# Ighina/MultimodalTopicSegmentation

Hardware: NVIDIA B200
Metric: segmented sentences/sec (higher is better)
Workload: dtype f32

## Files before the change

### include/mts_b200.h

```cpp
#ifndef MTS_B200_H_
#define MTS_B200_H_

#include <stdint.h>

#ifdef __cplusplus
extern "C" {
#endif

#define MTS_E_BADARG (-1)
#define MTS_E_UNSUPPORTED (-2)
#define MTS_E_NODEVICE (-3)

int mts_version(void);
const char *mts_last_error(void);
int mts_device_ok(void);


int mts_pack_rows_split(const float *src1, int64_t bstride1, int D1, const float *src2, int64_t bstride2, int D2,
                        int B, int T, int Kp, float *hi, float *lo, void *stream);

int mts_split_tf32(const float *src, int64_t ld, int rows, int cols, int Kp, int side, float *hi, float *lo,
                   void *stream);

int mts_transpose_split(const float *src, int64_t bstride, int64_t ld, int rows, int cols, int T, int shift,
                        const int32_t *lengths, int Kp, int side, float *hi, float *lo, void *stream);

int mts_gather_pad(const float *src, const int64_t *offsets, const int32_t *lengths, const int32_t *ids, int B, int T,
                   int D, float pad, float *out, void *stream);

int mts_ragged_copy(const float *src, float *dst, const int32_t *lengths, const int32_t *offsets, int B, int S, int d,
                    int to_padded, float pad, void *stream);

int mts_gemm_tf32x3(const float *A_hi, const float *A_lo, const float *B_hi, const float *B_lo, const float *bias,
                    float *C, int M, int N, int Kp, int64_t ldc, int epilogue, int accumulate, void *stream);
int mts_gemm_f32(const float *A, int64_t lda, const float *B, int64_t ldb, const float *bias, float *C, int64_t ldc,
                 int M, int N, int K, int layout, int epilogue, int accumulate, int splits, int shift, int T,
                 const int32_t *lengths, void *stream);
int64_t mts_colsum_ws_bytes(int M, int N);
int mts_colsum(const float *X, int64_t ld, int M, int N, float *out, int accumulate, void *ws, void *stream);

int mts_lstm_rec_fwd(const float *gx, const float *w_hh, const int32_t *lengths, const int32_t *order, int n_enc,
                     int B, int T, int H, float *y, float *gates, void *stream);

int mts_lstm_rec_fwd_tc(const float *gx, const float *w_hh, const int32_t *lengths, const int32_t *order, int n_enc,
                        int B, int T, int H, float *y, float *gates, float *y_corr, void *stream);
int mts_lstm_rec_fwd_tf32(const float *gx, const float *w_hh, const int32_t *lengths, const int32_t *order, int n_enc,
                          int B, int T, int H, float *y, float *gates, float *y_corr, void *stream);

int mts_gemm_tf32x3_srcs(const float *A1, int D1, int64_t ld1, const float *A2, int D2, int64_t ld2, const float *A_lo,
                         const float *B_hi, const float *B_lo, const float *bias, float *C, int M, int N, int Kp, int64_t ldc,
                         int epilogue, int accumulate, void *stream);

int mts_pack_rows_f16(const float *src1, int64_t bstride1, int D1, const float *src2, int64_t bstride2, int D2, int B, int T,
                      int K64, void *pieces, float *row_scale, void *stream);
int mts_gemm_f16x3(const void *A_pieces, const void *B_pieces, const float *row_scale, const float *col_scale, const float *bias,
                   float *C, float *C_lo, int M, int N, int K, int64_t ldc, int epilogue, void *stream);

int mts_gemm_tf32x3_gelu_pair(const float *A_hi, const float *A_lo, const float *B_hi, const float *B_lo, const float *bias,
                              float *C, float *C_lo, int M, int N, int Kp, void *stream);

int mts_lstm_rec_fwd_tc_bf16(const float *gx, const float *w_hh, const int32_t *lengths, const int32_t *order, int n_enc,
                             int B, int T, int H, float *y, float *gates, float *y_corr, void *stream);
int mts_gemm_bf16p(const float *A_lo, const float *B_lo, const float *bias, float *C, int M, int N, int Kp, int64_t ldc,
                   int epilogue, int accumulate, void *stream);
int mts_pack_rows_bf16in(const void *src1, int64_t bstride1, int D1, const void *src2, int64_t bstride2, int D2, int B, int T,
                         int Kp, float *lo, void *stream);

int mts_debug_rec_profile(long long *buf);

int mts_lstm_rec_fwd_h3(const float *gx, const float *w_hh, const int32_t *lengths, const int32_t *order, int n_enc,
                        int B, int T, int H, float *y, float *gates, float *y_corr, int precision, void *stream);
int mts_debug_rec_profile_h3(long long *buf);

int mts_lstm_rec_fwd_h3p(const float *gx, const float *w_hh, const int32_t *lengths, const int32_t *order, int n_enc,
                         int B, int T, int H, float *y, float *gates, float *y_corr, int precision, void *stream);
int mts_debug_rec_profile_h3p(long long *buf);

int mts_lstm_rec_bwd(const float *dy, const float *gates, const float *w_hh, const float *w_hh_t,
                     const int32_t *lengths, const int32_t *order, int n_enc, int B, int T, int H, float *dgx,
                     void *stream);

int mts_lstm_rec_bwd_tc(const float *dy, const float *gates, const float *w_hh, const int32_t *lengths,
                        const int32_t *order, int n_enc, int B, int T, int H, float *dgx, void *stream);
int mts_lstm_rec_bwd_h3(const float *dy, const float *gates, const float *w_hh, const int32_t *lengths,
                        const int32_t *order, int n_enc, int B, int T, int H, float *dgx, void *stream);
int mts_lstm_rec_bwd_tf32(const float *dy, const float *gates, const float *w_hh, const int32_t *lengths,
                          const int32_t *order, int n_enc, int B, int T, int H, float *dgx, void *stream);

int mts_head_fwd(const float *feats, const float *w, const float *bias, const int32_t *lengths, int B, int T, int F,
                 int n_out, float th, float *scores, uint8_t *tags, void *stream);
int64_t mts_head_bwd_ws_bytes(int B, int T, int F, int n_out);
int mts_head_bwd(const float *d_scores, const float *feats, const float *w, int B, int T, int F, int n_out,
                 float *d_feats, float *d_w, float *d_bias, void *ws, void *stream);

int mts_seg_loss_fwd(const float *scores, const float *target, int64_t ldt, const int32_t *lengths, int B, int T,
                     int kind, float alpha, float gamma, float inv_count, float *loss_out, float *partial,
                     void *stream);
int mts_seg_loss_bwd(const float *scores, const float *target, int64_t ldt, const int32_t *lengths, int B, int T,
                     int kind, float alpha, float gamma, float inv_count, const float *count_dev,
                     const float *grad_out, float *d_scores, void *stream);

int mts_seg_metrics(const uint8_t *tags, int64_t ld_tags, const float *target, int64_t ldt, const int32_t *lengths,
                    int B, int T, int zero_last, int32_t *out, void *stream);

int mts_crf_viterbi(const float *emis, const int32_t *lengths, const float *trans, int B, int L, int C,
                    float *best_score, int32_t *paths, uint32_t *bp_ws, void *stream);
int mts_crf_nll_fwd(const float *emis, const float *tags, int64_t ldt, const int32_t *lengths, const float *trans,
                    int B, int L, int C, float *log_z, float *gold, float *alphas, void *stream);
int mts_crf_nll_bwd(const float *emis, const float *tags, int64_t ldt, const int32_t *lengths, const float *trans,
                    const float *alphas, int B, int L, int C, const float *scale_dev, float *d_emis,
                    float *d_trans, void *stream);

int mts_embed_ln_fwd(const float *x, int64_t x_bstride, const float *pos, const float *typ, const float *gamma,
                     const float *beta, int B, int S, int d, float eps, float *y, float *y_hi, float *y_lo, int Kp,
                     float *sum_out, float *stats, const int32_t *lengths, const int32_t *offsets, void *stream);
int mts_add_ln_fwd(const float *a, const float *res, const float *gamma, const float *beta, int M, int d, float eps,
                   float *y, float *y_hi, float *y_lo, int Kp, float *sum_out, float *stats, void *stream);
int mts_embed_ln_fwd_f16(const float *x, int64_t x_bstride, const float *pos, const float *typ, const float *gamma,
                         const float *beta, int B, int S, int d, float eps, float *y, void *pieces, int K64, float *row_scale,
                         const int32_t *lengths, const int32_t *offsets, void *stream);
int mts_add_ln_fwd_f16(const float *a, const float *res, const float *gamma, const float *beta, int M, int d, float eps, float *y,
                       void *pieces, int K64, float *row_scale, void *stream);
int mts_gelu_split(const float *src, int64_t ld, int rows, int cols, int Kp, float *act, float *hi, float *lo,
                   void *stream);
// ... 37 lines not shown
```

### multimodaltopicsegmentation_b200/_lib.py

```python
from __future__ import annotations

import ctypes
import os
from ctypes import c_float, c_int, c_int64, c_uint64, c_void_p

_HERE = os.path.dirname(os.path.abspath(__file__))
LIB_PATH = os.path.join(_HERE, "libmts_b200.so")
CSRC = os.path.join(_HERE, "csrc")

_P = c_void_p

SIGNATURES = {
    "mts_version": (c_int, []),
    "mts_last_error": (ctypes.c_char_p, []),
    "mts_device_ok": (c_int, []),
    "mts_pack_rows_split": (c_int, [_P, c_int64, c_int, _P, c_int64, c_int, c_int, c_int, c_int, _P, _P, _P]),
    "mts_split_tf32": (c_int, [_P, c_int64, c_int, c_int, c_int, c_int, _P, _P, _P]),
    "mts_transpose_split": (c_int, [_P, c_int64, c_int64, c_int, c_int, c_int, c_int, _P, c_int, c_int, _P, _P, _P]),
    "mts_gather_pad": (c_int, [_P, _P, _P, _P, c_int, c_int, c_int, c_float, _P, _P]),
    "mts_gemm_tf32x3": (c_int, [_P, _P, _P, _P, _P, _P, c_int, c_int, c_int, c_int64, c_int, c_int, _P]),
    "mts_gemm_f32": (c_int, [_P, c_int64, _P, c_int64, _P, _P, c_int64, c_int, c_int, c_int, c_int, c_int, c_int,
                             c_int, c_int, c_int, _P, _P]),
    "mts_colsum_ws_bytes": (c_int64, [c_int, c_int]),
    "mts_colsum": (c_int, [_P, c_int64, c_int, c_int, _P, c_int, _P, _P]),
    "mts_lstm_rec_fwd": (c_int, [_P, _P, _P, _P, c_int, c_int, c_int, c_int, _P, _P, _P]),
    "mts_lstm_rec_fwd_tc": (c_int, [_P, _P, _P, _P, c_int, c_int, c_int, c_int, _P, _P, _P, _P]),
    "mts_lstm_rec_fwd_tc_bf16": (c_int, [_P, _P, _P, _P, c_int, c_int, c_int, c_int, _P, _P, _P, _P]),
    "mts_lstm_rec_fwd_tf32": (c_int, [_P, _P, _P, _P, c_int, c_int, c_int, c_int, _P, _P, _P, _P]),
    "mts_lstm_rec_fwd_h3": (c_int, [_P, _P, _P, _P, c_int, c_int, c_int, c_int, _P, _P, _P, c_int, _P]),
    "mts_gemm_tf32x3_srcs": (c_int, [_P, c_int, c_int64, _P, c_int, c_int64, _P, _P, _P, _P, _P, c_int, c_int, c_int, c_int64, c_int,
                                     c_int, _P]),
    "mts_pack_rows_f16": (c_int, [_P, c_int64, c_int, _P, c_int64, c_int, c_int, c_int, c_int, _P, _P, _P]),
    "mts_gemm_f16x3": (c_int, [_P, _P, _P, _P, _P, _P, _P, c_int, c_int, c_int, c_int64, c_int, _P]),
    "mts_gemm_tf32x3_gelu_pair": (c_int, [_P, _P, _P, _P, _P, _P, _P, c_int, c_int, c_int, _P]),
    "mts_gemm_bf16p": (c_int, [_P, _P, _P, _P, c_int, c_int, c_int, c_int64, c_int, c_int, _P]),
    "mts_pack_rows_bf16in": (c_int, [_P, c_int64, c_int, _P, c_int64, c_int, c_int, c_int, c_int, _P, _P]),
    "mts_debug_rec_profile": (c_int, [_P]),
    "mts_debug_rec_profile_h3": (c_int, [_P]),
    "mts_lstm_rec_fwd_h3p": (c_int, [_P, _P, _P, _P, c_int, c_int, c_int, c_int, _P, _P, _P, c_int, _P]),
    "mts_debug_rec_profile_h3p": (c_int, [_P]),
    "mts_lstm_rec_bwd": (c_int, [_P, _P, _P, _P, _P, _P, c_int, c_int, c_int, c_int, _P, _P]),
    "mts_lstm_rec_bwd_tc": (c_int, [_P, _P, _P, _P, _P, c_int, c_int, c_int, c_int, _P, _P]),
    "mts_lstm_rec_bwd_h3": (c_int, [_P, _P, _P, _P, _P, c_int, c_int, c_int, c_int, _P, _P]),
    "mts_lstm_rec_bwd_tf32": (c_int, [_P, _P, _P, _P, _P, c_int, c_int, c_int, c_int, _P, _P]),
    "mts_head_fwd": (c_int, [_P, _P, _P, _P, c_int, c_int, c_int, c_int, c_float, _P, _P, _P]),
    "mts_head_bwd_ws_bytes": (c_int64, [c_int, c_int, c_int, c_int]),
    "mts_head_bwd": (c_int, [_P, _P, _P, c_int, c_int, c_int, c_int, _P, _P, _P, _P, _P]),
    "mts_seg_loss_fwd": (c_int, [_P, _P, c_int64, _P, c_int, c_int, c_int, c_float, c_float, c_float, _P, _P, _P]),
    "mts_seg_loss_bwd": (c_int, [_P, _P, c_int64, _P, c_int, c_int, c_int, c_float, c_float, c_float, _P, _P, _P, _P]),
    "mts_seg_metrics": (c_int, [_P, c_int64, _P, c_int64, _P, c_int, c_int, c_int, _P, _P]),
    "mts_crf_viterbi": (c_int, [_P, _P, _P, c_int, c_int, c_int, _P, _P, _P, _P]),
    "mts_crf_nll_fwd": (c_int, [_P, _P, c_int64, _P, _P, c_int, c_int, c_int, _P, _P, _P, _P]),
    "mts_crf_nll_bwd": (c_int, [_P, _P, c_int64, _P, _P, _P, c_int, c_int, c_int, _P, _P, _P, _P]),
    "mts_embed_ln_fwd": (c_int, [_P, c_int64, _P, _P, _P, _P, c_int, c_int, c_int, c_float, _P, _P, _P, c_int, _P, _P, _P, _P,
                                 _P]),
    "mts_embed_ln_fwd_f16": (c_int, [_P, c_int64, _P, _P, _P, _P, c_int, c_int, c_int, c_float, _P, _P, c_int, _P, _P, _P, _P]),
    "mts_add_ln_fwd_f16": (c_int, [_P, _P, _P, _P, c_int, c_int, c_float, _P, _P, c_int, _P, _P]),
    "mts_add_ln_fwd": (c_int, [_P, _P, _P, _P, c_int, c_int, c_float, _P, _P, _P, c_int, _P, _P, _P]),
    "mts_gelu_split": (c_int, [_P, c_int64, c_int, c_int, c_int, _P, _P, _P, _P]),
    "mts_band_attn_fwd": (c_int, [_P, c_int64, _P, _P, c_int, c_int, c_int, c_int, c_int, _P, _P, _P, c_int, _P, _P]),
    "mts_band_attn_fwd_mma": (c_int, [_P, c_int64, _P, _P, c_int, c_int, c_int, c_int, c_int, _P, _P, _P, c_int, _P, _P]),
    "mts_band_attn_fwd_simt": (c_int, [_P, c_int64, _P, _P, c_int, c_int, c_int, c_int, c_int, _P, _P, _P, c_int, _P, _P]),
    "mts_band_attn_fwd_tc": (c_int, [_P, c_int64, _P, _P, c_int, c_int, c_int, c_int, c_int, _P, _P, _P, c_int, _P, _P]),
    "mts_band_attn_tc_supported": (c_int, [c_int]),
    "mts_debug_attn_profile": (c_int, [_P]),
    "mts_ln_bwd_ws_bytes": (c_int64, [c_int, c_int]),
    "mts_ln_bwd": (c_int, [_P, _P, _P, _P, c_int, c_int, _P, _P, _P, c_int, _P, _P, _P, _P]),
    "mts_gelu_bwd": (c_int, [_P, _P, c_int, c_int, c_int, _P, _P, _P, _P]),
    "mts_ragged_copy": (c_int, [_P, _P, _P, _P, c_int, c_int, c_int, c_int, c_float, _P]),
    "mts_embed_bwd": (c_int, [_P, c_int, c_int, c_int, _P, _P, _P, _P]),
    "mts_band_attn_bwd": (c_int, [_P, c_int64, _P, _P, _P, _P, _P, c_int, c_int, c_int, c_int, c_int, _P, _P, _P]),
    "mts_band_attn_fwd_dropout": (c_int, [_P, c_int64, _P, _P, c_int, c_int, c_int, c_int, c_int, _P, _P, _P, c_int, _P, c_float,
                                          c_uint64, _P]),
    "mts_band_attn_bwd_dropout": (c_int, [_P, c_int64, _P, _P, _P, _P, _P, c_int, c_int, c_int, c_int, c_int, _P, _P, c_float,
                                          c_uint64, _P]),
}

_lib = None


class MtsError(RuntimeError):
    pass
# ... 33 lines not shown
```

### multimodaltopicsegmentation_b200/csrc/gemm_tc.cu

```cuda
#include <cuda.h>
#include <stdlib.h>

#include "common.cuh"

namespace mts {

constexpr int TC_BM = 128;
constexpr int TC_BK = 32;
constexpr int TC_UMMA_K = 8;
constexpr int TC_THREADS = 192;

template <int BN>
struct TcCfg {
  static constexpr int kStages = (BN == 256) ? 2 : 3;
  static constexpr int kABytes = TC_BM * TC_BK * 4;
  static constexpr int kBBytes = BN * TC_BK * 4;
  static constexpr int kStageBytes = 2 * kABytes + 2 * kBBytes;
  static constexpr int kTmemCols = 2 * BN;
  static constexpr int kAccStride = BN;
  static constexpr int kSmemBytes = kStages * kStageBytes + 1024  + 256  + 4 * 32 * 32 * 4 ;
};

__device__ __forceinline__ uint32_t s_u32(const void *p) { return (uint32_t)__cvta_generic_to_shared(p); }

// ... 648 lines not shown
  static EncodeTiledFn fn = nullptr;
  if (!fn) {
    void *p = nullptr;
    cudaDriverEntryPointQueryResult q;
    if (cudaGetDriverEntryPoint("cuTensorMapEncodeTiled", &p, cudaEnableDefault, &q) == cudaSuccess &&
        q == cudaDriverEntryPointSuccess)
      fn = (EncodeTiledFn)p;
  }
  return fn;
}

static int make_map(CUtensorMap *map, const float *ptr, int rows, int Kp, int box_rows, bool corr = false, int cols = 0,
                    int64_t ld = 0) {
  EncodeTiledFn fn = get_encode_fn();
  if (!fn) { set_error("gemm_tf32x3: cuTensorMapEncodeTiled not available"); return MTS_E_NODEVICE; }
  if (cols == 0) cols = Kp;
  if (ld == 0) ld = Kp;
  cuuint64_t dims[2] = {(cuuint64_t)(corr ? 2 * cols : cols), (cuuint64_t)rows};
  cuuint64_t strides[1] = {(cuuint64_t)ld * sizeof(float)};
  cuuint32_t box[2] = {(cuuint32_t)(corr ? 2 * TC_BK : TC_BK), (cuuint32_t)box_rows};
  cuuint32_t estr[2] = {1, 1};
  CUresult r = fn(map, corr ? CU_TENSOR_MAP_DATA_TYPE_BFLOAT16 : CU_TENSOR_MAP_DATA_TYPE_FLOAT32, 2, (void *)ptr, dims, strides, box, estr,
                  CU_TENSOR_MAP_INTERLEAVE_NONE, CU_TENSOR_MAP_SWIZZLE_128B, CU_TENSOR_MAP_L2_PROMOTION_L2_256B,
                  CU_TENSOR_MAP_FLOAT_OOB_FILL_NONE);
  if (r != CUDA_SUCCESS) { set_error("gemm_tf32x3: cuTensorMapEncodeTiled failed"); return MTS_E_BADARG; }
  return 0;
}

__global__ void __launch_bounds__(256) zero_matrix_kernel(float *__restrict__ C, int M, int N, int64_t ldc) {
  const int64_t total = (int64_t)M * N;
  for (int64_t i = (int64_t)blockIdx.x * blockDim.x + threadIdx.x; i < total; i += (int64_t)gridDim.x * blockDim.x)
    C[(i / N) * ldc + (i % N)] = 0.0f;
}

struct ASources {
  const float *a1; int d1; int64_t ld1;
  const float *a2; int d2; int64_t ld2;
};

template <int BN>
static int launch_tc(const float *A_hi, const float *A_lo, const float *B_hi, const float *B_lo, const float *bias,
                     float *C, int M, int N, int Kp, int64_t ldc, int epilogue, int accumulate, cudaStream_t st,
                     int bf16_only = 0, float *C_lo = nullptr, const ASources *srcs = nullptr, const float *row_scale = nullptr,
                     const float *col_scale = nullptr) {
  using Cfg = TcCfg<BN>;
  const int tiles_m1 = (M + TC_BM - 1) / TC_BM;
  static const char *force = getenv("MTS_GEMM_CLUSTER");
  int CL = tiles_m1 >= 2 ? 2 : 1;
  if (force) {
    const int want = atoi(force);
    if ((want == 1 || want == 2) && tiles_m1 >= want) CL = want;
  }
  static const char *two = getenv("MTS_GEMM_2SM");
  const bool use_2sm = BN == 256 && tiles_m1 >= 2 && !(two && atoi(two) == 0);
  if (use_2sm) CL = 2;
  static const char *bn2_env = getenv("MTS_GEMM_BN2");
  int bn = BN;
  if (use_2sm && !(bn2_env && atoi(bn2_env) == 256) && N % 256 != 0 && (N + 223) / 224 == (N + 255) / 256)
    bn = 224;
  const int tiles_n = (N + bn - 1) / bn;
  CUtensorMap ma_hi, ma_lo, mb_hi, mb_lo;
  int rc;
  CUtensorMap ma_hi2;
  int a_split_kb = 1 << 30;
  if (srcs) {
    if ((rc = make_map(&ma_hi, srcs->a1, M, Kp, TC_BM, false, srcs->d1, srcs->ld1))) return rc;
    ma_hi2 = ma_hi;
    if (srcs->a2) {
      if ((rc = make_map(&ma_hi2, srcs->a2, M, Kp, TC_BM, false, srcs->d2, srcs->ld2))) return rc;
      a_split_kb = srcs->d1 / TC_BK;
    }
  } else {
    if ((rc = make_map(&ma_hi, A_hi, M, Kp, TC_BM, bf16_only == 2, 0, bf16_only == 2 ? 2 * Kp : 0))) return rc;
    ma_hi2 = ma_hi;
  }
  if ((rc = make_map(&ma_lo, A_lo, M, Kp, TC_BM, true, 0, bf16_only == 2 ? 2 * Kp : 0))) return rc;
  if ((rc = make_map(&mb_hi, B_hi, N, Kp, bn / CL, bf16_only == 2, 0, bf16_only == 2 ? 2 * Kp : 0))) return rc;
  if ((rc = make_map(&mb_lo, B_lo, N, Kp, bn / CL, true, 0, bf16_only == 2 ? 2 * Kp : 0))) return rc;
  MTS_PER_DEVICE(bool, attr_set);
  if (!attr_set) {
    MTS_CUDA(cudaFuncSetAttribute(gemm_tf32x3_kernel<BN, 1>, cudaFuncAttributeMaxDynamicSharedMemorySize, Cfg::kSmemBytes));
    MTS_CUDA(cudaFuncSetAttribute(gemm_tf32x3_kernel<BN, 2>, cudaFuncAttributeMaxDynamicSharedMemorySize, Cfg::kSmemBytes));
    MTS_CUDA(cudaFuncSetAttribute(gemm_tf32x3_2sm_kernel<256>, cudaFuncAttributeMaxDynamicSharedMemorySize, Tc2Cfg<256>::kSmemBytes));
    MTS_CUDA(cudaFuncSetAttribute(gemm_tf32x3_2sm_kernel<224>, cudaFuncAttributeMaxDynamicSharedMemorySize, Tc2Cfg<224>::kSmemBytes));
    attr_set = true;
  }
  const int tiles = ((tiles_m1 + CL - 1) / CL) * tiles_n;
  const int slots = kNumSMs / CL;
  int splits = 1;
  const int num_kb = Kp / TC_BK;
  if (epilogue != 2 && !C_lo) {
    if (tiles * 2 <= slots && num_kb >= 32) {
      splits = slots / tiles;
      if (splits > num_kb / 8) splits = num_kb / 8;
    }
    if (num_kb > 96 && splits < (num_kb + 63) / 64) splits = (num_kb + 63) / 64;
    if (splits < 1) splits = 1;
  }
  if (splits > 1 && !accumulate) {
    const int64_t total = (int64_t)M * N;
    const unsigned zg = (unsigned)((total + 255) / 256 < 1184 ? (total + 255) / 256 : 1184);
    zero_matrix_kernel<<<zg, 256, 0, st>>>(C, M, N, ldc);
  }
  const int items = tiles * splits;
  const int grid = (items < slots ? items : slots) * CL;
  cudaLaunchConfig_t cfg = {};
  cfg.gridDim = dim3((unsigned)grid);
// ... 105 lines not shown
```

### multimodaltopicsegmentation_b200/csrc/lstm_rec_h3.cu

```cuda
#include <cooperative_groups.h>
#include <cuda_fp16.h>
#include <stdlib.h>

#include "cluster_utils.cuh"
#include "tcgen05_utils.cuh"

namespace cg = cooperative_groups;

namespace mts {

constexpr int HR_NB = 16;
constexpr int HR_SUB_THREADS = 160;
constexpr int HR_EPI = 128;
constexpr int HR_PIECE_BYTES = 4 * HR_NB * 128;
constexpr int HR_B_BYTES = 2 * HR_PIECE_BYTES;
constexpr int HR_ACT_FLOATS = 4 * HR_NB * 32;
constexpr int HR_TMEM_COLS = 512;
constexpr int HR_W2_COL = 128;
constexpr int HR_ACC_COL = 256;
constexpr int HR_SUB_BYTES = 2 * HR_B_BYTES + HR_ACT_FLOATS * 4 + 1024;
constexpr int HR_HEAD_BYTES = 1024;
static_assert(HR_SUB_BYTES % 1024 == 0, "SWIZZLE_128B operand buffers need 1024-byte alignment");
template <int NT>
constexpr int hr_smem() {
  return (HR_HEAD_BYTES + NT * HR_SUB_BYTES + 1024) > 120 * 1024 ? (HR_HEAD_BYTES + NT * HR_SUB_BYTES + 1024) : 120 * 1024;
}

__host__ __device__ constexpr uint32_t idesc_f16(int M, int N) {
  return (1u << 4) | ((uint32_t)(N >> 3) << 17) | ((uint32_t)(M >> 4) << 24);
}

__device__ __forceinline__ uint32_t h2_bits(float first, float second) {
  const __half2 h = __floats2half2_rn(first, second);
  return *reinterpret_cast<const uint32_t *>(&h);
}
__device__ __forceinline__ float2 h2_floats(uint32_t bits) {
  return __half22float2(*reinterpret_cast<const __half2 *>(&bits));
}
__device__ __forceinline__ void st_async_v4u(uint32_t raddr, uint4 v, uint32_t rbar) {
  asm volatile("st.async.weak.shared::cluster.mbarrier::complete_tx::bytes.v4.b32 [%0], {%1, %2, %3, %4}, [%5];" ::"r"(raddr),
               "r"(v.x), "r"(v.y), "r"(v.z), "r"(v.w), "r"(rbar)
               : "memory");
}
__device__ __forceinline__ void tmem_st16u(uint32_t taddr, const uint32_t (&v)[16]) {
  asm volatile(
      "tcgen05.st.sync.aligned.32x32b.x16.b32 [%0], "
      "{%1, %2, %3, %4, %5, %6, %7, %8, %9, %10, %11, %12, %13, %14, %15, %16};" ::"r"(taddr),
      "r"(v[0]), "r"(v[1]), "r"(v[2]), "r"(v[3]), "r"(v[4]), "r"(v[5]), "r"(v[6]), "r"(v[7]), "r"(v[8]), "r"(v[9]), "r"(v[10]),
      "r"(v[11]), "r"(v[12]), "r"(v[13]), "r"(v[14]), "r"(v[15])
      : "memory");
}

__device__ __forceinline__ void umma_f16_ts_p(uint32_t d_tmem, uint32_t a_tmem, uint32_t b_lo, uint32_t b_hi, uint32_t idesc,
                                              uint32_t acc) {
  asm volatile(
      "{\n\t.reg .pred p;\n\t.reg .b64 bd;\n\t"
      "setp.ne.b32 p, %5, 0;\n\t"
      "mov.b64 bd, {%2, %3};\n\t"
      "tcgen05.mma.cta_group::1.kind::f16 [%0], [%1], bd, %4, p;\n\t}" ::"r"(d_tmem),
      "r"(a_tmem), "r"(b_lo), "r"(b_hi), "r"(idesc), "r"(acc)
      : "memory");
}

constexpr int HR_PROF_STEPS = 4, HR_PROF_SLOTS = 16;
__device__ long long *g_hr_prof = nullptr;
#define HR_STAMP(slot)                                                                     \
  do {                                                                                     \
    if (prof && s >= 8 && s < 8 + HR_PROF_STEPS) prof[(s - 8) * HR_PROF_SLOTS + (slot)] = clock64(); \
  } while (0)

template <bool SAVE, int NT, bool BF16>
__global__ void __cluster_dims__(kCluster, 1, 1) __launch_bounds__(HR_SUB_THREADS * NT, 1)
    lstm_fwd_h3_kernel(const float *__restrict__ gx, const float *__restrict__ w_hh, const int32_t *__restrict__ lengths,
                       const int32_t *__restrict__ order, int B, int T, int n_enc, int n_tiles, int ept,
                       float *__restrict__ y, float *__restrict__ gates, float *__restrict__ y_corr) {
  constexpr bool bf16_mode = BF16;
  extern __shared__ uint8_t smem_raw[];
  uint8_t *smem = reinterpret_cast<uint8_t *>((reinterpret_cast<uintptr_t>(smem_raw) + 1023) & ~(uintptr_t)1023);
  const int tid = threadIdx.x, lane = tid & 31;
  const int warp = __shfl_sync(0xffffffffu, tid >> 5, 0);
  const int sub = (NT == 2 && warp >= 5) ? 1 : 0;
  const int wr = warp - 5 * sub;

  float *rscale_s = reinterpret_cast<float *>(smem);
  uint32_t *tmem_slot = reinterpret_cast<uint32_t *>(smem + 512);
  uint8_t *sub_base = smem + HR_HEAD_BYTES + sub * HR_SUB_BYTES;
  uint8_t *bbuf = sub_base;
  float *act = reinterpret_cast<float *>(bbuf + 2 * HR_B_BYTES);
  uint64_t *bars = reinterpret_cast<uint64_t *>(act + HR_ACT_FLOATS);
  uint64_t *h_full = bars;
  uint64_t *acc_full = bars + 16;
  int *len_s = reinterpret_cast<int *>(bars + 18);
  int *bq_s = len_s + HR_NB;

  cg::cluster_group cluster = cg::this_cluster();
  const uint32_t rank = cluster.block_rank();
  const int n_clusters = gridDim.x / kCluster;
  const int groups = (n_tiles + NT - 1) / NT;
  const int n_items = groups * 2 * n_enc;
  const int ycols = n_enc * 2 * kH;

  if (wr == 0 && lane == 0) {
    for (int i = 0; i < 4; ++i) tc::bar_init(tc::s_u32(&h_full[i]), 1);
    tc::bar_init(tc::s_u32(acc_full), 1);
    asm volatile("fence.mbarrier_init.release.cluster;" ::: "memory");
  }
  if (warp == 0) tc::tmem_alloc<HR_TMEM_COLS>(tc::s_u32(tmem_slot));
  tc::tc_fence_before();
  __syncthreads();
  tc::tc_fence_after();
  const uint32_t tmem_base = *tmem_slot;
  const uint32_t acc_col = HR_ACC_COL + 16 * sub;

  uint32_t ph_h = 0, ph_acc = 0;

  const int et = (wr - 1) * 32 + lane;
  const int q = warp & 3;
  const int cj = et & 7, ce = et >> 3;

  int cur_dir = -1, cur_enc = -1;
  long long *prof = (blockIdx.x == 0 && (tid == 0 || tid == 32)) ? g_hr_prof : nullptr;

  for (int item = blockIdx.x / kCluster; item < n_items; item += n_clusters) {
    const int tile = (item % groups) * NT + sub;
    const int dir = (item / groups) & 1;
    const int enc = item / (2 * groups);
    const float *W = w_hh + ((size_t)enc * 2 + dir) * 4 * kH * kH;

// ... 127 lines not shown
      for (int i = 0; i < kCluster; ++i) {
        const uint32_t r = (rank + i) & 7;
        const uint32_t off = (uint32_t)(piece * HR_PIECE_BYTES + (i >> 1) * (HR_NB * 128) + ce * 128 +
                                        ((((i & 1) * 4 + chunk) ^ (ce & 7)) << 4));
        raddr[i] = mapa(tc::s_u32(bbuf) + off, r);
        rbar[i] = mapa(tc::s_u32(&h_full[i >> 2]), r);
      }
      const bool sender = ce < ept && !(bf16_mode && piece);

      for (int s = 0; s < nsteps; ++s) {
        const int p = s & 1;
        float gxc[HR_NB];
#pragma unroll
        for (int e = 0; e < HR_NB; ++e) {
          gxc[e] = gxn[e];
          const int len = len_s[e];
          if (s + 1 < len) {
            const int tn = dir ? len - 2 - s : s + 1;
            gxn[e] = __ldg(gx + gx_enc + ((size_t)bq_s[e] * T + tn) * 8 * kH + gcol);
          }
        }
        tc::bar_wait_wd(tc::s_u32(acc_full), ph_acc); ph_acc ^= 1;
        HR_STAMP(10);
        tc::tc_fence_after();
        float pre[HR_NB];
        tc::tmem_ld16(tmem_base + ((uint32_t)(q * 32) << 16) + acc_col, pre);
        tc::tc_fence_before();
        HR_STAMP(11);
        const float zs = (q == 2) ? -2.0f * 1.4426950408889634f : -1.4426950408889634f;
        const float oa = (q == 2) ? 2.0f : 1.0f, ob = (q == 2) ? -1.0f : 0.0f;
#define HR_ACT(NCOL)                                                          \
  _Pragma("unroll") for (int e = 0; e < (NCOL); ++e) {                        \
    const float z = fmaf(pre[e], rs, gxc[e]);                                 \
    const float sg = __fdividef(1.0f, 1.0f + exp2f(z * zs));                  \
    act[(q * HR_NB + e) * 32 + lane] = fmaf(sg, oa, ob);                      \
  }
        if (ept > 14) { HR_ACT(16) } else if (ept > 12) { HR_ACT(14) } else if (ept > 10) { HR_ACT(12) } else if (ept > 8) { HR_ACT(10) }
        else if (ept > 6) { HR_ACT(8) } else if (ept > 4) { HR_ACT(6) } else if (ept > 2) { HR_ACT(4) } else { HR_ACT(2) }
#undef HR_ACT
        if (sub == 0) asm volatile("bar.sync 1, 128;" ::: "memory");
        else asm volatile("bar.sync 2, 128;" ::: "memory");
        HR_STAMP(12);
        const float4 ig = *reinterpret_cast<const float4 *>(act + (0 * HR_NB + ce) * 32 + 4 * cj);
        const float4 fg = *reinterpret_cast<const float4 *>(act + (1 * HR_NB + ce) * 32 + 4 * cj);
        const float4 gg = *reinterpret_cast<const float4 *>(act + (2 * HR_NB + ce) * 32 + 4 * cj);
        const float4 og = *reinterpret_cast<const float4 *>(act + (3 * HR_NB + ce) * 32 + 4 * cj);
        float4 hn = make_float4(0.f, 0.f, 0.f, 0.f);
        if (s < my_len) {
          c[0] = fmaf(fg.x, c[0], ig.x * gg.x); c[1] = fmaf(fg.y, c[1], ig.y * gg.y);
          c[2] = fmaf(fg.z, c[2], ig.z * gg.z); c[3] = fmaf(fg.w, c[3], ig.w * gg.w);
          hn = make_float4(og.x * tanh_fast(c[0]), og.y * tanh_fast(c[1]), og.z * tanh_fast(c[2]), og.w * tanh_fast(c[3]));
        }
        HR_STAMP(13);
        if (s + 1 < nsteps) {
          uint32_t p1a, p1b, p2a = 0u, p2b = 0u;
          if (bf16_mode) {
            p1a = bf16x2_bits(hn.x, hn.y);
            p1b = bf16x2_bits(hn.z, hn.w);
          } else {
            p1a = h2_bits(hn.x, hn.y);
            p1b = h2_bits(hn.z, hn.w);
            const float2 f0 = h2_floats(p1a), f1 = h2_floats(p1b);
            p2a = h2_bits(hn.x - f0.x, hn.y - f0.y);
            p2b = h2_bits(hn.z - f1.x, hn.w - f1.y);
          }
          const uint32_t ga = piece ? p1a : p2a, gb = piece ? p1b : p2b;
          const uint32_t ra = __shfl_xor_sync(0xffffffffu, ga, 1), rb = __shfl_xor_sync(0xffffffffu, gb, 1);
          const uint4 gran = piece ? make_uint4(ra, rb, p2a, p2b) : make_uint4(p1a, p1b, ra, rb);
          if (sender) {
            const uint32_t boff = (uint32_t)((p ^ 1) * HR_B_BYTES), moff = (uint32_t)((p ^ 1) * 16);
#pragma unroll
            for (int r = 0; r < kCluster; ++r) st_async_v4u(raddr[r] + boff, gran, rbar[r] + moff);
          }
        }
        HR_STAMP(14);
        if (s < my_len) {
          const int t = dir ? my_len - 1 - s : s;
          *reinterpret_cast<float4 *>(y + ((size_t)my_b * T + t) * ycols + ycol) = hn;
          if (y_corr) corr_store4(y_corr + ((size_t)my_b * T + t) * ycols, (int)ycol, hn, 0);
          if (SAVE) {
            float *gs = gates + ((gate_base + my_b) * T + t) * 5 * kH + rank * kUnits + 4 * cj;
            *reinterpret_cast<float4 *>(gs) = ig;
            *reinterpret_cast<float4 *>(gs + kH) = fg;
            *reinterpret_cast<float4 *>(gs + 2 * kH) = gg;
            *reinterpret_cast<float4 *>(gs + 3 * kH) = og;
            *reinterpret_cast<float4 *>(gs + 4 * kH) = make_float4(c[0], c[1], c[2], c[3]);
          }
        }
      }
      if (my_b >= 0)
        for (int t = my_len; t < T; ++t) {
          const float4 z = make_float4(0.f, 0.f, 0.f, 0.f);
          *reinterpret_cast<float4 *>(y + ((size_t)my_b * T + t) * ycols + ycol) = z;
          if (y_corr) corr_store4(y_corr + ((size_t)my_b * T + t) * ycols, (int)ycol, z, 0);
        }
    }
    tc::tc_fence_before();
    __syncthreads();
    cluster.sync();
  }
  tc::tc_fence_before();
  __syncthreads();
  if (warp == 0) {
    tc::tc_fence_after();
    tc::tmem_dealloc<HR_TMEM_COLS>(tmem_base);
  }
}

template <typename K>
static int h3_max_active_clusters(K kernel, int threads, int smem) {
  cudaLaunchConfig_t cfg = {};
  cfg.gridDim = dim3(kCluster * 64);
  cfg.blockDim = dim3(threads);
  cfg.dynamicSmemBytes = smem;
  cudaLaunchAttribute attr;
  attr.id = cudaLaunchAttributeClusterDimension;
  attr.val.clusterDim.x = kCluster;
  attr.val.clusterDim.y = 1;
  attr.val.clusterDim.z = 1;
  cfg.attrs = &attr;
  cfg.numAttrs = 1;
  int n = 0;
  if (cudaOccupancyMaxActiveClusters(&n, kernel, &cfg) != cudaSuccess || n < 1) {
    cudaGetLastError();
    n = 8;
  }
  return n;
}

}

using namespace mts;

extern "C" int mts_debug_rec_profile_h3(long long *buf) {
  MTS_CUDA(cudaMemcpyToSymbol(g_hr_prof, &buf, sizeof(buf)));
  return 0;
}

template <bool BF16>
static int launch_h3(const float *gx, const float *w_hh, const int32_t *lengths, const int32_t *order, int n_enc, int B, int T,
                     float *y, float *gates, float *y_corr, cudaStream_t st) {
  MTS_PER_DEVICE(int, cap);
  if (!cap) {
    MTS_CUDA(cudaFuncSetAttribute(lstm_fwd_h3_kernel<false, 1, BF16>, cudaFuncAttributeMaxDynamicSharedMemorySize, hr_smem<1>()));
    MTS_CUDA(cudaFuncSetAttribute(lstm_fwd_h3_kernel<true, 1, BF16>, cudaFuncAttributeMaxDynamicSharedMemorySize, hr_smem<1>()));
    MTS_CUDA(cudaFuncSetAttribute(lstm_fwd_h3_kernel<false, 2, BF16>, cudaFuncAttributeMaxDynamicSharedMemorySize, hr_smem<2>()));
    MTS_CUDA(cudaFuncSetAttribute(lstm_fwd_h3_kernel<true, 2, BF16>, cudaFuncAttributeMaxDynamicSharedMemorySize, hr_smem<2>()));
    cap = h3_max_active_clusters(lstm_fwd_h3_kernel<false, 2, BF16>, 2 * HR_SUB_THREADS, hr_smem<2>());
  }
  int ept = HR_NB;
  {
    const int per_dir = cap / (2 * n_enc);
    if (per_dir >= 1 && (B + HR_NB - 1) / HR_NB <= per_dir) {
      const int want = (B + per_dir - 1) / per_dir;
      ept = want < 1 ? 1 : (want > HR_NB ? HR_NB : want);
    }
  }
  static const char *force_ept = getenv("MTS_REC_EPT");
  if (force_ept && atoi(force_ept) >= 1 && atoi(force_ept) <= HR_NB) ept = atoi(force_ept);
  const int n_tiles = (B + ept - 1) / ept;
  const int items1 = n_tiles * 2 * n_enc;
  static const char *force = getenv("MTS_REC_NT");
  const bool two = force ? (force[0] == '2') : (items1 > cap);
  static const char *pair_env = getenv("MTS_REC_PAIR");
  if (pair_env ? (pair_env[0] == '1') : two)
    return mts_lstm_rec_fwd_h3p(gx, w_hh, lengths, order, n_enc, B, T, kH, y, gates, y_corr, BF16 ? 1 : 0, (void *)st);
  if (!two) {
    const unsigned grid = (unsigned)((items1 < cap ? items1 : cap) * kCluster);
    if (gates) lstm_fwd_h3_kernel<true, 1, BF16><<<grid, HR_SUB_THREADS, hr_smem<1>(), st>>>(gx, w_hh, lengths, order, B, T, n_enc, n_tiles, ept, y, gates, y_corr);
    else lstm_fwd_h3_kernel<false, 1, BF16><<<grid, HR_SUB_THREADS, hr_smem<1>(), st>>>(gx, w_hh, lengths, order, B, T, n_enc, n_tiles, ept, y, gates, y_corr);
  } else {
    const int items2 = ((n_tiles + 1) / 2) * 2 * n_enc;
    const unsigned grid = (unsigned)((items2 < cap ? items2 : cap) * kCluster);
    if (gates) lstm_fwd_h3_kernel<true, 2, BF16><<<grid, 2 * HR_SUB_THREADS, hr_smem<2>(), st>>>(gx, w_hh, lengths, order, B, T, n_enc, n_tiles, ept, y, gates, y_corr);
    else lstm_fwd_h3_kernel<false, 2, BF16><<<grid, 2 * HR_SUB_THREADS, hr_smem<2>(), st>>>(gx, w_hh, lengths, order, B, T, n_enc, n_tiles, ept, y, gates, y_corr);
  }
  MTS_LAUNCH_CHECK();
  return 0;
}

extern "C" int mts_lstm_rec_fwd_h3(const float *gx, const float *w_hh, const int32_t *lengths, const int32_t *order, int n_enc,
                                   int B, int T, int H, float *y, float *gates, float *y_corr, int precision, void *stream) {
  MTS_REQUIRE(gx && w_hh && lengths && y, MTS_E_BADARG, "lstm_rec_fwd_h3: null pointer");
  MTS_REQUIRE(n_enc >= 1 && B > 0 && T > 0, MTS_E_BADARG, "lstm_rec_fwd_h3: bad shape");
  MTS_REQUIRE(H == kH, MTS_E_UNSUPPORTED, "lstm_rec_fwd_h3: the tensor-core recurrence serves H == 256");
  MTS_REQUIRE(precision == 0 || precision == 1, MTS_E_BADARG, "lstm_rec_fwd_h3: precision must be 0 (fp16 x3) or 1 (bf16)");
  MTS_REQUIRE(!y_corr || n_enc == 1, MTS_E_UNSUPPORTED, "lstm_rec_fwd_h3: the fused correction operand needs n_enc == 1");
  MTS_REQUIRE((((uintptr_t)y | (uintptr_t)gx | (uintptr_t)w_hh) & 15) == 0, MTS_E_BADARG,
              "lstm_rec_fwd_h3: buffers must be 16-byte aligned");
  cudaStream_t st = (cudaStream_t)stream;
  return precision ? launch_h3<true>(gx, w_hh, lengths, order, n_enc, B, T, y, gates, y_corr, st)
                   : launch_h3<false>(gx, w_hh, lengths, order, n_enc, B, T, y, gates, y_corr, st);
}
```

### multimodaltopicsegmentation_b200/ops.py

```python
from __future__ import annotations

import torch

from . import _lib

_LAUNCHES = 0
_KERNELS_PER_CALL = {
    "mts_seg_loss_fwd": 2, "mts_head_bwd": 3, "mts_colsum": 2, "mts_ln_bwd": 3, "mts_band_attn_bwd": 2,
}


def launch_count():
    return _LAUNCHES


def reset_launch_count():
    global _LAUNCHES
    _LAUNCHES = 0


PROFILE = None
GEMM_IMPL = __import__("os").environ.get("MTS_GEMM_IMPL", "tcgen05")
REC_IMPL = __import__("os").environ.get("MTS_REC_IMPL", "tc")

# ... 311 lines not shown
        cache = ent.setdefault("wih_p", {})
        if e not in cache:
            w_f, _, _, _, w_r = self._params(self.rnns[e], layer)[:5]
            with torch.no_grad():
                cache[e] = f16_pieces_stacked([w_f.detach(), w_r.detach()])
        return cache[e]

    def wih_packed_a(self, layer, e):
        ent = self.get()[layer]
        cache = ent.setdefault("wih_bf", {})
        if e not in cache:
            w_f, _, _, _, w_r = self._params(self.rnns[e], layer)[:5]
            D = w_f.shape[1]
            kp = _pad32(D)
            H4 = w_f.shape[0]
            bf = torch.empty((2, 2 * H4, kp), device=w_f.device, dtype=torch.float32)
            with torch.no_grad():
                for d, w in enumerate((w_f, w_r)):
                    wc = w.detach().contiguous()
                    _call("mts_split_tf32", _ptr(wc), D, H4, D, kp, A_SIDE, _ptr(bf[0, d * H4:]), _ptr(bf[1, d * H4:]), _stream())
            cache[e] = bf[1]
        return cache[e]

    def get(self):
        key = tuple((p.data_ptr(), p._version) for p in self.flat_params())
        if key == self.key:
            return self.layers
        rnn0 = self.rnns[0]
        H, L = rnn0.hidden_size, rnn0.num_layers
        dev = rnn0.weight_hh_l0.device
        layers = []
        with torch.no_grad():
            for layer in range(L):
                wih, bias = [], []
                whh = torch.empty((len(self.rnns), 2, 4 * H, H), device=dev, dtype=torch.float32)
                for e, rnn in enumerate(self.rnns):
                    w_f, h_f, bi_f, bh_f, w_r, h_r, bi_r, bh_r = self._params(rnn, layer)
                    D = w_f.shape[1]
                    kp = _pad32(D)
                    pair = torch.empty((2, 8 * H, kp), device=dev, dtype=torch.float32)
                    for d, w in enumerate((w_f, w_r)):
                        wc = w.detach().contiguous()
                        _call("mts_split_tf32", _ptr(wc), D, 4 * H, D, kp, B_SIDE, _ptr(pair[0, d * 4 * H:]),
                              _ptr(pair[1, d * 4 * H:]), _stream())
                    wih.append((pair[0], pair[1]))
                    bias.append(torch.cat([bi_f.detach() + bh_f.detach(), bi_r.detach() + bh_r.detach()]))
                    whh[e, 0].copy_(h_f.detach())
                    whh[e, 1].copy_(h_r.detach())
                layers.append({"wih": wih, "bias": bias, "whh": whh})
        self.key, self.layers = key, layers
        return layers


def _lstm_stack_forward(x1, x2, xs2, lens, packed, H, L, n_enc, save):
    B, T = lens.B, lens.T
    dev = x1.device
    layers = packed.get()
    saved = []
    y_prev = y_corr = None
    bf16 = PRECISION == "bf16"
    if bf16 and (save or H != 256 or REC_IMPL != "tc" or GEMM_IMPL == "simt"):
        raise NotImplementedError("the bf16 path serves inference with H == 256 on the tensor-core kernels; train in fp32")
    for layer in range(L):
        gx = torch.empty((n_enc, B * T, 8 * H), device=dev, dtype=torch.float32)
        for e in range(n_enc):
            if bf16:
                if layer == 0:
                    a_lo = pack_rows_packed(x1, x2, B, T) if n_enc == 1 else pack_rows_packed(x1 if e == 0 else xs2, None, B, T)
                elif y_corr is not None:
                    a_lo = y_corr
                else:
                    src = y_prev.view(B * T, n_enc * 2 * H)[:, e * 2 * H:(e + 1) * 2 * H]
                    a_lo = split_tf32(src, cols=2 * H, ld=n_enc * 2 * H, rows=B * T)[1]
                _call("mts_gemm_bf16p", _ptr(a_lo), _ptr(packed.wih_packed_a(layer, e)), _ptr(layers[layer]["bias"][e]), _ptr(gx[e]),
                      B * T, 8 * H, a_lo.shape[1], 8 * H, 1, 0, _stream())
                continue
            if layer == 0 and GEMM_IMPL != "simt":
                w_hi, w_lo = layers[layer]["wih"][e]
                wp = lambda e=e: packed.wih_pieces(0, e)
                if n_enc == 1:
                    input_projection(x1, x2, B, T, w_hi, w_lo, layers[layer]["bias"][e], gx[e], 8 * H, w_pieces=wp)
                else:
                    input_projection(x1 if e == 0 else xs2, None, B, T, w_hi, w_lo, layers[layer]["bias"][e], gx[e], 8 * H,
                                     w_pieces=wp)
                continue
            if layer == 0:
                if n_enc == 1:
                    a_hi, a_lo = pack_rows_split(x1, x2, B, T)
                else:
                    a_hi, a_lo = pack_rows_split(x1 if e == 0 else xs2, None, B, T)
            elif y_corr is not None:
                a_hi, a_lo = y_prev.view(B * T, 2 * H), y_corr
            else:
                src = y_prev.view(B * T, n_enc * 2 * H)[:, e * 2 * H:(e + 1) * 2 * H]
                a_hi, a_lo = split_tf32(src, cols=2 * H, ld=n_enc * 2 * H, rows=B * T)
            w_hi, w_lo = layers[layer]["wih"][e]
            if GEMM_IMPL == "simt":
                a, w = a_hi, w_hi
                gemm_f32(_ptr(a), a.shape[1], _ptr(w), w.shape[1], layers[layer]["bias"][e], _ptr(gx[e]), 8 * H, B * T,
                         8 * H, a.shape[1], layout=0, epilogue=1)
            else:
                gemm_tf32x3(a_hi, a_lo, w_hi, w_lo, layers[layer]["bias"][e], gx[e], B * T, 8 * H, epilogue=1,
                            ldc=8 * H)
        y = torch.empty((B, T, n_enc * 2 * H), device=dev, dtype=torch.float32)
        gates = torch.empty((n_enc, 2, B, T, 5, H), device=dev, dtype=torch.float32) if save else None
        if H == 256 and REC_IMPL == "tc":
            y_corr = (torch.empty((B * T, 2 * H), device=dev, dtype=torch.float32)
                      if (n_enc == 1 and layer + 1 < L and GEMM_IMPL != "simt") else None)
            _call("mts_lstm_rec_fwd_tc_bf16" if bf16 else "mts_lstm_rec_fwd_tc", _ptr(gx), _ptr(layers[layer]["whh"]),
                  _ptr(lens.dev), _ptr(lens.order), n_enc, B, T, H, _ptr(y), _ptr(gates), _ptr(y_corr), _stream())
        else:
            y_corr = None
            _call("mts_lstm_rec_fwd", _ptr(gx), _ptr(layers[layer]["whh"]), _ptr(lens.dev), _ptr(lens.order), n_enc, B, T,
                  H, _ptr(y), _ptr(gates), _stream())
        saved.append((y_prev, y, gates))
        y_prev = y
    return y_prev, saved


def bilstm_stack(x1, x2, xs2, lens, packed, n_enc):
    x1, x2, xs2 = (_rows_ok(x1, "input", lens.B, lens.T), _rows_ok(x2, "second input", lens.B, lens.T),
                   _rows_ok(xs2, "second encoder input", lens.B, lens.T))
    flat = packed.flat_params()
    if not (torch.is_grad_enabled() and (any(p.requires_grad for p in flat) or x1.requires_grad)):
        rnn0 = packed.rnns[0]
        return _lstm_stack_forward(x1, x2, xs2, lens, packed, rnn0.hidden_size, rnn0.num_layers, n_enc, save=False)[0]
    return BiLstmStackFn.apply(x1, x2, xs2, lens, packed, n_enc, *flat)


class BiLstmStackFn(torch.autograd.Function):

    @staticmethod
    def forward(ctx, x1, x2, xs2, lens, packed, n_enc, *flat):
        rnn0 = packed.rnns[0]
        H, L = rnn0.hidden_size, rnn0.num_layers
        need = any(ctx.needs_input_grad)
        y, saved = _lstm_stack_forward(x1, x2, xs2, lens, packed, H, L, n_enc, save=need)
        if need:
            ctx.x1, ctx.x2, ctx.xs2, ctx.lens, ctx.packed, ctx.n_enc = x1, x2, xs2, lens, packed, n_enc
            ctx.saved = saved
            ctx.HL = (H, L)
        return y

    @staticmethod
    def backward(ctx, dy):
        H, L = ctx.HL
        lens, packed, n_enc = ctx.lens, ctx.packed, ctx.n_enc
        B, T = lens.B, lens.T
        N = B * T
        layers = packed.get()
        dev = dy.device
        dy = dy.contiguous()
        grads = [[None] * (8 * L) for _ in range(n_enc)]
        dx_in = None
        splits = max(1, min(16, N // 2048))
        tensor_core = GEMM_IMPL != "simt"
# ... 212 lines not shown
```

Baseline: 19.01 million.

## Emit fp16 hi/lo output pieces from LSTM recurrence to feed next-layer f16x3 GEMM

Adds a variant of the h3 forward recurrence that writes each hidden output as two fp16 pieces (hi and residual lo) directly in the layout the f16x3 GEMM consumes. For non-final layers in inference, the next layer's input projection then reads these pieces instead of an fp32 output that has to be split again. This removes the fp32 y/y_corr writes and the separate split pass, and halves the bytes written per output element. The fp16-pieces GEMM is forced onto the 2-SM path, the pair-kernel path is skipped, and the route only applies when the batch fits one wave and several other conditions hold.

New measurement: 19.59 million, median of 6. +3.1%, better.

```diff
diff --git a/include/mts_b200.h b/include/mts_b200.h
--- a/include/mts_b200.h
+++ b/include/mts_b200.h
@@ -70,6 +70,9 @@
 
 int mts_lstm_rec_fwd_h3(const float *gx, const float *w_hh, const int32_t *lengths, const int32_t *order, int n_enc,
                         int B, int T, int H, float *y, float *gates, float *y_corr, int precision, void *stream);
+int mts_lstm_rec_fwd_h3_f16y(const float *gx, const float *w_hh, const int32_t *lengths, const int32_t *order, int B, int T, int H,
+                             void *y_pieces, void *stream);
+int mts_lstm_rec_fwd_h3_f16y_max_batch(void);
 int mts_debug_rec_profile_h3(long long *buf);
 
 int mts_lstm_rec_fwd_h3p(const float *gx, const float *w_hh, const int32_t *lengths, const int32_t *order, int n_enc,
diff --git a/multimodaltopicsegmentation_b200/_lib.py b/multimodaltopicsegmentation_b200/_lib.py
--- a/multimodaltopicsegmentation_b200/_lib.py
+++ b/multimodaltopicsegmentation_b200/_lib.py
@@ -28,6 +28,8 @@
     "mts_lstm_rec_fwd_tc_bf16": (c_int, [_P, _P, _P, _P, c_int, c_int, c_int, c_int, _P, _P, _P, _P]),
     "mts_lstm_rec_fwd_tf32": (c_int, [_P, _P, _P, _P, c_int, c_int, c_int, c_int, _P, _P, _P, _P]),
     "mts_lstm_rec_fwd_h3": (c_int, [_P, _P, _P, _P, c_int, c_int, c_int, c_int, _P, _P, _P, c_int, _P]),
+    "mts_lstm_rec_fwd_h3_f16y": (c_int, [_P, _P, _P, _P, c_int, c_int, c_int, _P, _P]),
+    "mts_lstm_rec_fwd_h3_f16y_max_batch": (c_int, []),
     "mts_gemm_tf32x3_srcs": (c_int, [_P, c_int, c_int64, _P, c_int, c_int64, _P, _P, _P, _P, _P, c_int, c_int, c_int, c_int64, c_int,
                                      c_int, _P]),
     "mts_pack_rows_f16": (c_int, [_P, c_int64, c_int, _P, c_int64, c_int, c_int, c_int, c_int, _P, _P, _P]),
diff --git a/multimodaltopicsegmentation_b200/csrc/gemm_tc.cu b/multimodaltopicsegmentation_b200/csrc/gemm_tc.cu
--- a/multimodaltopicsegmentation_b200/csrc/gemm_tc.cu
+++ b/multimodaltopicsegmentation_b200/csrc/gemm_tc.cu
@@ -724,7 +724,8 @@
     if ((want == 1 || want == 2) && tiles_m1 >= want) CL = want;
   }
   static const char *two = getenv("MTS_GEMM_2SM");
-  const bool use_2sm = BN == 256 && tiles_m1 >= 2 && !(two && atoi(two) == 0);
+  const bool use_2sm = BN == 256 && tiles_m1 >= 2 && (bf16_only == 2 || !(two && atoi(two) == 0));
+  MTS_REQUIRE(use_2sm || bf16_only != 2, MTS_E_UNSUPPORTED, "gemm_f16x3: the fp16-split product needs M, N >= 256");
   if (use_2sm) CL = 2;
   static const char *bn2_env = getenv("MTS_GEMM_BN2");
   int bn = BN;
diff --git a/multimodaltopicsegmentation_b200/csrc/lstm_rec_h3.cu b/multimodaltopicsegmentation_b200/csrc/lstm_rec_h3.cu
--- a/multimodaltopicsegmentation_b200/csrc/lstm_rec_h3.cu
+++ b/multimodaltopicsegmentation_b200/csrc/lstm_rec_h3.cu
@@ -73,7 +73,8 @@
 __global__ void __cluster_dims__(kCluster, 1, 1) __launch_bounds__(HR_SUB_THREADS * NT, 1)
     lstm_fwd_h3_kernel(const float *__restrict__ gx, const float *__restrict__ w_hh, const int32_t *__restrict__ lengths,
                        const int32_t *__restrict__ order, int B, int T, int n_enc, int n_tiles, int ept,
-                       float *__restrict__ y, float *__restrict__ gates, float *__restrict__ y_corr) {
+                       float *__restrict__ y, float *__restrict__ gates, float *__restrict__ y_corr,
+                       uint16_t *__restrict__ y_pieces) {
   constexpr bool bf16_mode = BF16;
   extern __shared__ uint8_t smem_raw[];
   uint8_t *smem = reinterpret_cast<uint8_t *>((reinterpret_cast<uintptr_t>(smem_raw) + 1023) & ~(uintptr_t)1023);
@@ -307,18 +308,18 @@
           hn = make_float4(og.x * tanh_fast(c[0]), og.y * tanh_fast(c[1]), og.z * tanh_fast(c[2]), og.w * tanh_fast(c[3]));
         }
         HR_STAMP(13);
+        uint32_t p1a, p1b, p2a = 0u, p2b = 0u;
+        if (bf16_mode) {
+          p1a = bf16x2_bits(hn.x, hn.y);
+          p1b = bf16x2_bits(hn.z, hn.w);
+        } else {
+          p1a = h2_bits(hn.x, hn.y);
+          p1b = h2_bits(hn.z, hn.w);
+          const float2 f0 = h2_floats(p1a), f1 = h2_floats(p1b);
+          p2a = h2_bits(hn.x - f0.x, hn.y - f0.y);
+          p2b = h2_bits(hn.z - f1.x, hn.w - f1.y);
+        }
         if (s + 1 < nsteps) {
-          uint32_t p1a, p1b, p2a = 0u, p2b = 0u;
-          if (bf16_mode) {
-            p1a = bf16x2_bits(hn.x, hn.y);
-            p1b = bf16x2_bits(hn.z, hn.w);
-          } else {
-            p1a = h2_bits(hn.x, hn.y);
-            p1b = h2_bits(hn.z, hn.w);
-            const float2 f0 = h2_floats(p1a), f1 = h2_floats(p1b);
-            p2a = h2_bits(hn.x - f0.x, hn.y - f0.y);
-            p2b = h2_bits(hn.z - f1.x, hn.w - f1.y);
-          }
           const uint32_t ga = piece ? p1a : p2a, gb = piece ? p1b : p2b;
           const uint32_t ra = __shfl_xor_sync(0xffffffffu, ga, 1), rb = __shfl_xor_sync(0xffffffffu, gb, 1);
           const uint4 gran = piece ? make_uint4(ra, rb, p2a, p2b) : make_uint4(p1a, p1b, ra, rb);
@@ -331,8 +332,14 @@
         HR_STAMP(14);
         if (s < my_len) {
           const int t = dir ? my_len - 1 - s : s;
-          *reinterpret_cast<float4 *>(y + ((size_t)my_b * T + t) * ycols + ycol) = hn;
-          if (y_corr) corr_store4(y_corr + ((size_t)my_b * T + t) * ycols, (int)ycol, hn, 0);
+          if (y_pieces) {
+            uint16_t *yp = y_pieces + ((size_t)my_b * T + t) * 2 * ycols + ycol;
+            *reinterpret_cast<uint2 *>(yp) = make_uint2(p1a, p1b);
+            *reinterpret_cast<uint2 *>(yp + ycols) = make_uint2(p2a, p2b);
+          } else {
+            *reinterpret_cast<float4 *>(y + ((size_t)my_b * T + t) * ycols + ycol) = hn;
+            if (y_corr) corr_store4(y_corr + ((size_t)my_b * T + t) * ycols, (int)ycol, hn, 0);
+          }
           if (SAVE) {
             float *gs = gates + ((gate_base + my_b) * T + t) * 5 * kH + rank * kUnits + 4 * cj;
             *reinterpret_cast<float4 *>(gs) = ig;
@@ -346,6 +353,12 @@
       if (my_b >= 0)
         for (int t = my_len; t < T; ++t) {
           const float4 z = make_float4(0.f, 0.f, 0.f, 0.f);
+          if (y_pieces) {
+            uint16_t *yp = y_pieces + ((size_t)my_b * T + t) * 2 * ycols + ycol;
+            *reinterpret_cast<uint2 *>(yp) = make_uint2(0u, 0u);
+            *reinterpret_cast<uint2 *>(yp + ycols) = make_uint2(0u, 0u);
+            continue;
+          }
           *reinterpret_cast<float4 *>(y + ((size_t)my_b * T + t) * ycols + ycol) = z;
           if (y_corr) corr_store4(y_corr + ((size_t)my_b * T + t) * ycols, (int)ycol, z, 0);
         }
@@ -394,7 +407,7 @@
 
 template <bool BF16>
 static int launch_h3(const float *gx, const float *w_hh, const int32_t *lengths, const int32_t *order, int n_enc, int B, int T,
-                     float *y, float *gates, float *y_corr, cudaStream_t st) {
+                     float *y, float *gates, float *y_corr, cudaStream_t st, uint16_t *y_pieces = nullptr) {
   MTS_PER_DEVICE(int, cap);
   if (!cap) {
     MTS_CUDA(cudaFuncSetAttribute(lstm_fwd_h3_kernel<false, 1, BF16>, cudaFuncAttributeMaxDynamicSharedMemorySize, hr_smem<1>()));
@@ -418,17 +431,17 @@
   static const char *force = getenv("MTS_REC_NT");
   const bool two = force ? (force[0] == '2') : (items1 > cap);
   static const char *pair_env = getenv("MTS_REC_PAIR");
-  if (pair_env ? (pair_env[0] == '1') : two)
+  if (!y_pieces && (pair_env ? (pair_env[0] == '1') : two))
     return mts_lstm_rec_fwd_h3p(gx, w_hh, lengths, order, n_enc, B, T, kH, y, gates, y_corr, BF16 ? 1 : 0, (void *)st);
   if (!two) {
     const unsigned grid = (unsigned)((items1 < cap ? items1 : cap) * kCluster);
-    if (gates) lstm_fwd_h3_kernel<true, 1, BF16><<<grid, HR_SUB_THREADS, hr_smem<1>(), st>>>(gx, w_hh, lengths, order, B, T, n_enc, n_tiles, ept, y, gates, y_corr);
-    else lstm_fwd_h3_kernel<false, 1, BF16><<<grid, HR_SUB_THREADS, hr_smem<1>(), st>>>(gx, w_hh, lengths, order, B, T, n_enc, n_tiles, ept, y, gates, y_corr);
+    if (gates) lstm_fwd_h3_kernel<true, 1, BF16><<<grid, HR_SUB_THREADS, hr_smem<1>(), st>>>(gx, w_hh, lengths, order, B, T, n_enc, n_tiles, ept, y, gates, y_corr, y_pieces);
+    else lstm_fwd_h3_kernel<false, 1, BF16><<<grid, HR_SUB_THREADS, hr_smem<1>(), st>>>(gx, w_hh, lengths, order, B, T, n_enc, n_tiles, ept, y, gates, y_corr, y_pieces);
   } else {
     const int items2 = ((n_tiles + 1) / 2) * 2 * n_enc;
     const unsigned grid = (unsigned)((items2 < cap ? items2 : cap) * kCluster);
-    if (gates) lstm_fwd_h3_kernel<true, 2, BF16><<<grid, 2 * HR_SUB_THREADS, hr_smem<2>(), st>>>(gx, w_hh, lengths, order, B, T, n_enc, n_tiles, ept, y, gates, y_corr);
-    else lstm_fwd_h3_kernel<false, 2, BF16><<<grid, 2 * HR_SUB_THREADS, hr_smem<2>(), st>>>(gx, w_hh, lengths, order, B, T, n_enc, n_tiles, ept, y, gates, y_corr);
+    if (gates) lstm_fwd_h3_kernel<true, 2, BF16><<<grid, 2 * HR_SUB_THREADS, hr_smem<2>(), st>>>(gx, w_hh, lengths, order, B, T, n_enc, n_tiles, ept, y, gates, y_corr, y_pieces);
+    else lstm_fwd_h3_kernel<false, 2, BF16><<<grid, 2 * HR_SUB_THREADS, hr_smem<2>(), st>>>(gx, w_hh, lengths, order, B, T, n_enc, n_tiles, ept, y, gates, y_corr, y_pieces);
   }
   MTS_LAUNCH_CHECK();
   return 0;
@@ -447,3 +460,27 @@
   return precision ? launch_h3<true>(gx, w_hh, lengths, order, n_enc, B, T, y, gates, y_corr, st)
                    : launch_h3<false>(gx, w_hh, lengths, order, n_enc, B, T, y, gates, y_corr, st);
 }
+
+static int h3_one_wave_cap() {
+  MTS_PER_DEVICE(int, cap);
+  if (!cap) {
+    if (cudaFuncSetAttribute(lstm_fwd_h3_kernel<false, 2, false>, cudaFuncAttributeMaxDynamicSharedMemorySize, hr_smem<2>()) != cudaSuccess) {
+      cudaGetLastError();
+      return 0;
+    }
+    cap = h3_max_active_clusters(lstm_fwd_h3_kernel<false, 2, false>, 2 * HR_SUB_THREADS, hr_smem<2>());
+  }
+  return cap;
+}
+extern "C" int mts_lstm_rec_fwd_h3_f16y_max_batch(void) { return (h3_one_wave_cap() / 2) * HR_NB; }
+
+extern "C" int mts_lstm_rec_fwd_h3_f16y(const float *gx, const float *w_hh, const int32_t *lengths, const int32_t *order, int B, int T,
+                                        int H, void *y_pieces, void *stream) {
+  MTS_REQUIRE(gx && w_hh && lengths && y_pieces, MTS_E_BADARG, "lstm_rec_fwd_h3_f16y: null pointer");
+  MTS_REQUIRE(B > 0 && T > 0, MTS_E_BADARG, "lstm_rec_fwd_h3_f16y: bad shape");
+  MTS_REQUIRE(H == kH, MTS_E_UNSUPPORTED, "lstm_rec_fwd_h3_f16y: the tensor-core recurrence serves H == 256");
+  MTS_REQUIRE((((uintptr_t)y_pieces | (uintptr_t)gx | (uintptr_t)w_hh) & 15) == 0, MTS_E_BADARG,
+              "lstm_rec_fwd_h3_f16y: buffers must be 16-byte aligned");
+  return launch_h3<false>(gx, w_hh, lengths, order, 1, B, T, nullptr, nullptr, nullptr, (cudaStream_t)stream,
+                          reinterpret_cast<uint16_t *>(y_pieces));
+}
diff --git a/multimodaltopicsegmentation_b200/ops.py b/multimodaltopicsegmentation_b200/ops.py
--- a/multimodaltopicsegmentation_b200/ops.py
+++ b/multimodaltopicsegmentation_b200/ops.py
@@ -387,12 +387,25 @@
         return layers
 
 
+_F16Y_MAX_B = {}
+
+
+def _f16y_ok(B, T, H, n_enc, save, last):
+    if (save or last or n_enc != 1 or H != 256 or PRECISION == "bf16" or REC_IMPL != "tc" or GEMM_IMPL == "simt" or not PROJ_F16X3
+            or B * T < 256 or __import__("os").environ.get("MTS_REC_TC", "").startswith("t")):
+        return False
+    d = torch.cuda.current_device()
+    if d not in _F16Y_MAX_B:
+        _F16Y_MAX_B[d] = _lib.load().mts_lstm_rec_fwd_h3_f16y_max_batch()
+    return B <= _F16Y_MAX_B[d]
+
+
 def _lstm_stack_forward(x1, x2, xs2, lens, packed, H, L, n_enc, save):
     B, T = lens.B, lens.T
     dev = x1.device
     layers = packed.get()
     saved = []
-    y_prev = y_corr = None
+    y_prev = y_corr = y_pieces = None
     bf16 = PRECISION == "bf16"
     if bf16 and (save or H != 256 or REC_IMPL != "tc" or GEMM_IMPL == "simt"):
         raise NotImplementedError("the bf16 path serves inference with H == 256 on the tensor-core kernels; train in fp32")
@@ -419,6 +432,10 @@
                     input_projection(x1 if e == 0 else xs2, None, B, T, w_hi, w_lo, layers[layer]["bias"][e], gx[e], 8 * H,
                                      w_pieces=wp)
                 continue
+            if y_pieces is not None:
+                wp, ws = packed.wih_pieces(layer, e)
+                gemm_f16x3(y_pieces, None, wp, ws, layers[layer]["bias"][e], gx[e], B * T, 8 * H, epilogue=1)
+                continue
             if layer == 0:
                 if n_enc == 1:
                     a_hi, a_lo = pack_rows_split(x1, x2, B, T)
@@ -437,6 +454,15 @@
             else:
                 gemm_tf32x3(a_hi, a_lo, w_hi, w_lo, layers[layer]["bias"][e], gx[e], B * T, 8 * H, epilogue=1,
                             ldc=8 * H)
+        if _f16y_ok(B, T, H, n_enc, save, layer + 1 == L):
+            y = y_corr = None
+            y_pieces = torch.empty((B * T, 2, 2 * H), device=dev, dtype=torch.float16)
+            _call("mts_lstm_rec_fwd_h3_f16y", _ptr(gx), _ptr(layers[layer]["whh"]), _ptr(lens.dev), _ptr(lens.order), B, T, H,
+                  _ptr(y_pieces), _stream())
+            saved.append((y_prev, y, None))
+            y_prev = y
+            continue
+        y_pieces = None
         y = torch.empty((B, T, n_enc * 2 * H), device=dev, dtype=torch.float32)
         gates = torch.empty((n_enc, 2, B, T, 5, H), device=dev, dtype=torch.float32) if save else None
         if H == 256 and REC_IMPL == "tc":
```
